# nkb-tech/nkb-classification

Hardware: AMD Instinct MI355X
Metric: images/sec train step (3x224x224) (higher is better)
Workload: dtype bf16; 1 GPU; resnet50 single-task train step, 1000 classes, bs=256/GPU, bf16 compute + fp32 master weights, NAdam, 3x224x224; global_batch=256, parallelism=dp1

## Files before the change

nkb-classification_amd/csrc/elementwise.hip:

```cpp
#include "common.h"
#include <stdlib.h>
#include <atomic>

static inline unsigned grid_for(size_t work_items, int block = 256, unsigned cap = 256 * 16) {
    size_t g = (work_items + block - 1) / block;
    if (g > cap) g = cap;
    if (g < 1) g = 1;
    return (unsigned)g;
}

template <typename T> struct Chunk;
template <> struct Chunk<bf16_t> {
    static constexpr int N = 8;
    typedef u32x4 Raw;
    __device__ static __forceinline__ Raw ldraw(const bf16_t* p) { return *(const u32x4*)p; }
    __device__ static __forceinline__ void unpack(const Raw& r, float* f) { unpack8(r, f); }
    __device__ static __forceinline__ void load(const bf16_t* p, float* f) { unpack8(*(const u32x4*)p, f); }
    __device__ static __forceinline__ void store(bf16_t* p, const float* f) { *(u32x4*)p = pack8(f); }
};
template <> struct Chunk<float> {
    static constexpr int N = 4;
    typedef f32x4 Raw;
    __device__ static __forceinline__ Raw ldraw(const float* p) { return *(const f32x4*)p; }
    __device__ static __forceinline__ void unpack(const Raw& r, float* f) { f[0] = r[0]; f[1] = r[1]; f[2] = r[2]; f[3] = r[3]; }
    __device__ static __forceinline__ void load(const float* p, float* f) {
        const f32x4 v = *(const f32x4*)p;
        f[0] = v[0]; f[1] = v[1]; f[2] = v[2]; f[3] = v[3];
    }
    __device__ static __forceinline__ void store(float* p, const float* f) { *(f32x4*)p = (f32x4){f[0], f[1], f[2], f[3]}; }
};

static inline int env_int(const char* name, int dflt) {
    const char* v = getenv(name);
    return v && *v ? atoi(v) : dflt;
}
#ifndef NKB_BN_FUSED
#define NKB_BN_FUSED 1
#endif
static constexpr int g_bn_fused = NKB_BN_FUSED;

template <int NC>
__device__ __forceinline__ void ldvec(const float* __restrict__ p, float* o) {
#pragma unroll
    for (int i = 0; i < NC / 4; ++i) {
        const f32x4 v = *(const f32x4*)(p + 4 * i);
        o[4 * i] = v[0]; o[4 * i + 1] = v[1]; o[4 * i + 2] = v[2]; o[4 * i + 3] = v[3];
    }
}

static inline int bn_partitions(int C) { return C <= 128 ? 64 : (C <= 256 ? 32 : 16); }
template <bool WT>
__device__ __forceinline__ void bn_partial_reduce_body(const float* __restrict__ partials, int tiles, int C, double* __restrict__ dpart,
                                                       double (&red)[2][16][64]) {
    const int cx = threadIdx.x & 63, py = threadIdx.x >> 6;
    const int c = blockIdx.x * 64 + cx;
    double s = 0.0, ss = 0.0;
    if (c < C) {
        for (int t = blockIdx.y * 16 + py; t < tiles; t += 16 * (int)gridDim.y) {
            s += (double)partials[((size_t)t * 2) * C + c];
            ss += (double)partials[((size_t)t * 2 + 1) * C + c];
        }
    }
    red[0][py][cx] = s;
    red[1][py][cx] = ss;
    __syncthreads();
    if (py != 0 || c >= C) return;
    s = 0.0; ss = 0.0;
    for (int k = 0; k < 16; ++k) { s += red[0][k][cx]; ss += red[1][k][cx]; }
    double* d0 = dpart + ((size_t)blockIdx.y * 2) * C + c;
    double* d1 = dpart + ((size_t)blockIdx.y * 2 + 1) * C + c;
    if constexpr (WT) {
        __hip_atomic_store(d0, s, __ATOMIC_RELAXED, __HIP_MEMORY_SCOPE_AGENT);
        __hip_atomic_store(d1, ss, __ATOMIC_RELAXED, __HIP_MEMORY_SCOPE_AGENT);
    } else {
        *d0 = s; *d1 = ss;
    }
}
__global__ void bn_partial_reduce_kernel(const float* __restrict__ partials, int tiles, int C, double* __restrict__ dpart) {
    __shared__ double red[2][16][64];
    bn_partial_reduce_body<false>(partials, tiles, C, dpart, red);
}

__device__ unsigned g_bn_tickets[128 * 32];
__device__ __forceinline__ bool bn_arrive_last(unsigned* ticket, unsigned parts) {
    __shared__ unsigned last_flag;
    asm volatile("s_waitcnt vmcnt(0)" ::: "memory");
    __syncthreads();
    if (threadIdx.x == 0) {
        const unsigned t = __hip_atomic_fetch_add(ticket, 1u, __ATOMIC_RELAXED, __HIP_MEMORY_SCOPE_AGENT);
        const bool last = t == parts - 1;
        if (last) {
            __hip_atomic_store(ticket, 0u, __ATOMIC_RELAXED, __HIP_MEMORY_SCOPE_AGENT);
            __builtin_amdgcn_fence(__ATOMIC_ACQUIRE, "agent");
            asm volatile("s_waitcnt vmcnt(0)" ::: "memory");
        }
        last_flag = last ? 1u : 0u;
    }
    __syncthreads();
    return last_flag != 0u;
}
static unsigned* bn_ticket_slot(int cols) {
    static std::atomic<unsigned> next{0};
    if (cols > 32) return nullptr;
    unsigned* base = nullptr;
    if (hipGetSymbolAddress((void**)&base, HIP_SYMBOL(g_bn_tickets)) != hipSuccess || !base) return nullptr;
    return base + (next.fetch_add(1u) % 128u) * 32u;
}

template <typename PT>
__device__ __forceinline__ void bn_finalize_body(const PT* __restrict__ partials, int tiles, int C, float count,
                                                 const float* __restrict__ gamma, const float* __restrict__ beta,
                                                 float* __restrict__ running_mean, float* __restrict__ running_var,
                                                 float momentum, float eps, int training, float* __restrict__ scale,
                                                 float* __restrict__ shift, float* __restrict__ save_mean,
                                                 float* __restrict__ save_invstd, double (&red)[2][16][64]) {
    const int cx = threadIdx.x & 63, py = threadIdx.x >> 6;
    const int c = blockIdx.x * 64 + cx;
    double s = 0.0, ss = 0.0;
    if (training && c < C) {
        for (int t = py; t < tiles; t += 16) {
            s += (double)partials[((size_t)t * 2) * C + c];
            ss += (double)partials[((size_t)t * 2 + 1) * C + c];
        }
    }
    red[0][py][cx] = s;
    red[1][py][cx] = ss;
    __syncthreads();
    if (py != 0 || c >= C) return;
    float mean, var;
    if (training) {
        s = 0.0; ss = 0.0;
        for (int k = 0; k < 16; ++k) { s += red[0][k][cx]; ss += red[1][k][cx]; }
        const double m = s / count;
        double v = ss / count - m * m;
        if (v < 0.0) v = 0.0;
        mean = (float)m; var = (float)v;
        const float unbiased = count > 1.f ? (float)(v * count / (count - 1.0)) : var;
        running_mean[c] = (1.f - momentum) * running_mean[c] + momentum * mean;
        running_var[c] = (1.f - momentum) * running_var[c] + momentum * unbiased;
    } else {
        mean = running_mean[c]; var = running_var[c];
    }
    const float invstd = 1.0f / sqrtf(var + eps);
    const float g = gamma ? gamma[c] : 1.f, b = beta ? beta[c] : 0.f;
    scale[c] = g * invstd;
    shift[c] = b - mean * g * invstd;
    if (save_mean) { save_mean[c] = mean; save_invstd[c] = invstd; }
}
template <typename PT>
__global__ void bn_finalize_kernel(const PT* __restrict__ partials, int tiles, int C, float count,
                                   const float* __restrict__ gamma, const float* __restrict__ beta,
                                   float* __restrict__ running_mean, float* __restrict__ running_var,
                                   float momentum, float eps, int training, float* __restrict__ scale,
                                   float* __restrict__ shift, float* __restrict__ save_mean,
                                   float* __restrict__ save_invstd) {
    __shared__ double red[2][16][64];
    bn_finalize_body<PT>(partials, tiles, C, count, gamma, beta, running_mean, running_var, momentum, eps, training, scale, shift,
                         save_mean, save_invstd, red);
}
__global__ __launch_bounds__(1024) void bn_reduce_finalize_kernel(const float* __restrict__ partials, int tiles, int C, double* __restrict__ dpart,
// ... 1276 lines not shown
    const int cx = threadIdx.x & 63, py = threadIdx.x >> 6;
    const int c = blockIdx.x * 64 + cx;
    double a = 0.0, b = 0.0;
    if (c < C) {
        for (int t = py; t < tiles; t += 16) {
            a += (double)partials[((size_t)t * 2) * C + c];
            b += (double)partials[((size_t)t * 2 + 1) * C + c];
        }
    }
    red[0][py][cx] = a;
    red[1][py][cx] = b;
    __syncthreads();
    if (py != 0 || c >= C) return;
    a = 0.0; b = 0.0;
    for (int k = 0; k < 16; ++k) { a += red[0][k][cx]; b += red[1][k][cx]; }
    const float sg = (float)a, sgx = (float)(b * (invstd ? (double)invstd[c] : 1.0));
    sums[c] = sg;
    sums[C + c] = sgx;
    if (dbeta) dbeta[c] += sg;
    if (dgamma) dgamma[c] += sgx;
}
template <typename PT>
__global__ void bn_bwd_finalize_tiles_kernel(const PT* __restrict__ partials, int tiles, int C,
                                             const float* __restrict__ invstd, float* __restrict__ dgamma,
                                             float* __restrict__ dbeta, float* __restrict__ sums) {
    __shared__ double red[2][16][64];
    bn_bwd_finalize_tiles_body<PT>(partials, tiles, C, invstd, dgamma, dbeta, sums, red);
}
__global__ __launch_bounds__(1024) void bn_bwd_reduce_finalize_kernel(const float* __restrict__ stats, int tiles, int C, double* __restrict__ dpart,
                                                                      unsigned* __restrict__ tickets, const float* __restrict__ invstd,
                                                                      float* __restrict__ dgamma, float* __restrict__ dbeta,
                                                                      float* __restrict__ sums) {
    __shared__ double red[2][16][64];
    bn_partial_reduce_body<true>(stats, tiles, C, dpart, red);
    if (!bn_arrive_last(tickets + blockIdx.x, gridDim.y)) return;
    bn_bwd_finalize_tiles_body<double>(dpart, (int)gridDim.y, C, invstd, dgamma, dbeta, sums, red);
}

static void launch_bwd_tile_sums(float* stats, int tiles, int C, const float* invstd, float* dgamma, float* dbeta, float* sums,
                                 hipStream_t stream) {
    double* dpart = (double*)(stats + (((size_t)tiles * 2 * C + 1) & ~(size_t)1));
    const int P = bn_partitions(C);
    unsigned* tickets = g_bn_fused ? bn_ticket_slot((C + 63) / 64) : nullptr;
    if (tickets) {
        hipLaunchKernelGGL(bn_bwd_reduce_finalize_kernel, dim3((C + 63) / 64, P), dim3(1024), 0, stream, stats, tiles, C, dpart, tickets,
                           invstd, dgamma, dbeta, sums);
        return;
    }
    hipLaunchKernelGGL(bn_partial_reduce_kernel, dim3((C + 63) / 64, P), dim3(1024), 0, stream, stats, tiles, C, dpart);
    hipLaunchKernelGGL(bn_bwd_finalize_tiles_kernel<double>, dim3((C + 63) / 64), dim3(1024), 0, stream,
                       (const double*)dpart, P, C, invstd, dgamma, dbeta, sums);
}

int nkb_launch_tile_sums(float* stats, int tiles, int C, float* sums, hipStream_t stream) {
    if (tiles > 128) {
        launch_bwd_tile_sums(stats, tiles, C, nullptr, nullptr, nullptr, sums, stream);
    } else {
        hipLaunchKernelGGL(bn_bwd_finalize_tiles_kernel<float>, dim3((C + 63) / 64), dim3(1024), 0, stream,
                           (const float*)stats, tiles, C, (const float*)nullptr, (float*)nullptr, (float*)nullptr, sums);
    }
    return nkb_check_launch("tile_sums");
}

extern "C" int nkb_bn_backward_from_stats(int dtype, const void* g, const void* x, float* stats, int tiles,
                                          const float* mean, const float* invstd, const float* gamma, long long rows,
                                          int C, float* dgamma, float* dbeta, void* dx, float* sums, hipStream_t stream) {
    const int n = dtype == NKB_DT_BF16 ? 8 : 4;
    if (C % n || rows >= (1ll << 31)) { nkb_set_error("bn_backward_from_stats: unsupported C=%d / rows", C); return 1; }
    {
        NkbProfScope prof(NKB_K_BN_BWD_REDUCE, stream, 0);
        if (tiles > 128) {
            launch_bwd_tile_sums(stats, tiles, C, invstd, dgamma, dbeta, sums, stream);
        } else {
            hipLaunchKernelGGL(bn_bwd_finalize_tiles_kernel<float>, dim3((C + 63) / 64), dim3(1024), 0, stream,
                               (const float*)stats, tiles, C, invstd, dgamma, dbeta, sums);
        }
    }
    if (int rc = nkb_check_launch("bn_bwd_finalize_tiles")) return rc;
    NkbProfScope prof(NKB_K_BN_BWD_APPLY, stream, 0, (double)rows * C * (dtype == NKB_DT_BF16 ? 2 : 4) * 3);
    const unsigned grid = grid_cols((size_t)rows, C / n);
    if (dtype == NKB_DT_BF16)
        hipLaunchKernelGGL(bn_bwd_apply_kernel<bf16_t>, dim3(grid), dim3(256), 0, stream, (const bf16_t*)g, (const bf16_t*)x,
                           (const bf16_t*)nullptr, (const unsigned char*)nullptr, (const float*)nullptr, (const float*)nullptr, mean, invstd, gamma, sums,
                           1.0f / (float)rows, (unsigned)rows, C, (bf16_t*)dx, (bf16_t*)nullptr);
    else
        hipLaunchKernelGGL(bn_bwd_apply_kernel<float>, dim3(grid), dim3(256), 0, stream, (const float*)g, (const float*)x,
                           (const float*)nullptr, (const unsigned char*)nullptr, (const float*)nullptr, (const float*)nullptr, mean, invstd, gamma, sums,
                           1.0f / (float)rows, (unsigned)rows, C, (float*)dx, (float*)nullptr);
    return nkb_check_launch("bn_bwd_apply");
}
```

nkb-classification_amd/csrc/grambn.hip:

```cpp
#include "common.h"
#include "prims.h"
#include <stdlib.h>

template <typename WT> __device__ __forceinline__ float ldw(const WT* p);
template <> __device__ __forceinline__ float ldw<float>(const float* p) { return *p; }
template <> __device__ __forceinline__ float ldw<bf16_t>(const bf16_t* p) { return bf2f(*p); }

int nkb_launch_tile_sums(float* stats, int tiles, int C, float* sums, hipStream_t stream);


template <int C>
__global__ __launch_bounds__(256, 3) void bn_apply_gram_kernel(const bf16_t* __restrict__ c, bf16_t* __restrict__ y,
                                                               const float* __restrict__ scale, const float* __restrict__ shift,
                                                               unsigned rows, float* __restrict__ part) {
    constexpr int CPR = C / 8;
    constexpr int RPS = 256 / CPR;
    constexpr int SR = 8192 / C;
    constexpr int NP = SR / RPS;
    constexpr int NBLK = C / 16, NB = NBLK / 2;
    extern __shared__ __attribute__((aligned(16))) unsigned char smem[];
    const int tid = threadIdx.x, lane = tid & 63, wave = tid >> 6;
    const int wr = wave >> 1, wn = wave & 1;
    const int cc = tid % CPR, srow = tid / CPR;
    float sc[8], sh[8], bsum[8];
    {
        const f32x4 a0 = *(const f32x4*)(scale + cc * 8), a1 = *(const f32x4*)(scale + cc * 8 + 4);
        const f32x4 b0 = *(const f32x4*)(shift + cc * 8), b1 = *(const f32x4*)(shift + cc * 8 + 4);
#pragma unroll
        for (int e = 0; e < 4; ++e) { sc[e] = a0[e]; sc[4 + e] = a1[e]; sh[e] = b0[e]; sh[4 + e] = b1[e]; }
    }
#pragma unroll
    for (int e = 0; e < 8; ++e) bsum[e] = 0.f;
    f32x4 acc[NB][NB];
#pragma unroll
    for (int i = 0; i < NB; ++i)
#pragma unroll
        for (int j = 0; j < NB; ++j) acc[i][j] = (f32x4){0.f, 0.f, 0.f, 0.f};
    const unsigned nstage = (rows + SR - 1) / SR;
    u32x4 ld[NP];
    auto load = [&](unsigned st) {
#pragma unroll
        for (int i = 0; i < NP; ++i) {
            const unsigned r = st * SR + srow + RPS * i;
            ld[i] = (u32x4){0u, 0u, 0u, 0u};
            if (r < rows) ld[i] = *(const u32x4*)(c + (size_t)r * C + cc * 8);
        }
    };
    const int g = lane >> 4, li = lane & 15, q4 = li >> 2, p4 = li & 3;
    unsigned st = blockIdx.x;
    if (st < nstage) load(st);
    for (; st < nstage; st += gridDim.x) {
#pragma unroll
        for (int i = 0; i < NP; ++i) {
            const unsigned r = st * SR + srow + RPS * i;
            float v[8];
            unpack8(ld[i], v);
#pragma unroll
            for (int e = 0; e < 8; ++e) v[e] = fmaxf(v[e] * sc[e] + sh[e], 0.f);
            u32x4 pk = pack8(v);
            if (r < rows) { if (y) *(u32x4*)(y + (size_t)r * C + cc * 8) = pk; }
            else pk = (u32x4){0u, 0u, 0u, 0u};
// ... 183 lines not shown
            }
        }
        __syncthreads();
#pragma unroll
        for (int ii = 0; ii < IC; ++ii) {
            const f32x4 w4 = *(const f32x4*)(wl + (size_t)(i0 + ii < Cin ? i0 + ii : 0) * KR);
            const float w[KR] = {w4[0], w4[1], w4[2], w4[3]};
#pragma unroll
            for (int jj = 0; jj < NJ; ++jj) {
                const int j = tid + 256 * jj;
                const float cv = j < Cin ? cl[(size_t)ii * Cin + j] : 0.f;
#pragma unroll
                for (int k = 0; k < KR; ++k) acc[k][jj] += w[k] * cv;
            }
        }
    }
    float pv[KR], pm[KR];
#pragma unroll
    for (int k = 0; k < KR; ++k) { pv[k] = 0.f; pm[k] = 0.f; }
#pragma unroll
    for (int jj = 0; jj < NJ; ++jj) {
        const int j = tid + 256 * jj;
        if (j < Cin) {
            const float mj = mu[j];
#pragma unroll
            for (int k = 0; k < KR; ++k) {
                if (k0 + k < Cout) T[(size_t)(k0 + k) * Cin + j] = acc[k][jj];
                pv[k] += acc[k][jj] * wl[j * KR + k];
                pm[k] += wl[j * KR + k] * mj;
            }
        }
    }
    float var[KR], mean[KR];
    block_sums<KR>(pv, red, var);
    block_sums<KR>(pm, red, mean);
    if (tid < KR && k0 + tid < Cout) {
        const int c = k0 + tid;
        float v = 0.f, m = 0.f;
#pragma unroll
        for (int k = 0; k < KR; ++k) if (k == tid) { v = var[k]; m = mean[k]; }
        if (v < 0.f) v = 0.f;
        const float unbiased = count > 1.f ? v * (count / (count - 1.f)) : v;
        running_mean[c] = (1.f - momentum) * running_mean[c] + momentum * m;
        running_var[c] = (1.f - momentum) * running_var[c] + momentum * unbiased;
        const float invstd = 1.0f / sqrtf(v + eps);
        const float g = gamma ? gamma[c] : 1.f, b = beta ? beta[c] : 0.f;
        scale[c] = g * invstd;
        shift[c] = b - m * g * invstd;
        save_mean[c] = m;
        save_invstd[c] = invstd;
    }
}

template <typename WT, typename CT, int NJ>
__global__ __launch_bounds__(256) void gram_bwd_coef_kernel(const WT* __restrict__ W, const float* __restrict__ R,
                                                            const float* __restrict__ T, const float* __restrict__ mu,
                                                            const float* __restrict__ gsum, float count, int Cin, int Cout,
                                                            const float* __restrict__ gamma, const float* __restrict__ mean,
                                                            const float* __restrict__ invstd, float* __restrict__ dgamma,
                                                            float* __restrict__ dbeta, float* __restrict__ dW,
                                                            CT* __restrict__ wcat, int ldc, CT* __restrict__ V,
                                                            float* __restrict__ cpart) {
    constexpr int KR = 8;
    __shared__ float red[4 * KR];
    __shared__ float kc[5][KR];
    const int tid = threadIdx.x;
    const int k0 = blockIdx.x * KR;
    float w[KR][NJ], r[KR][NJ], p[KR];
#pragma unroll
    for (int k = 0; k < KR; ++k) {
        p[k] = 0.f;
#pragma unroll
        for (int jj = 0; jj < NJ; ++jj) {
            const int j = tid + 256 * jj;
            const bool ok = j < Cin && k0 + k < Cout;
            w[k][jj] = ok ? ldw<WT>(W + (size_t)(k0 + k) * Cin + j) : 0.f;
            r[k][jj] = ok ? R[(size_t)(k0 + k) * Cin + j] : 0.f;
            p[k] += w[k][jj] * r[k][jj];
        }
    }
    float gc[KR];
    block_sums<KR>(p, red, gc);
    if (tid < KR) {
        const int c = k0 + tid;
        float s = 0.f;
#pragma unroll
        for (int k = 0; k < KR; ++k) if (k == tid) s = gc[k];
        float k1 = 0.f, k2 = 0.f, k3 = 0.f, gb = 0.f;
        if (c < Cout) {
            const float g = gamma ? gamma[c] : 1.f, rs = invstd[c], m = mean[c], db = gsum[c];
            const float dg = rs * (s - m * db);
            k1 = g * rs;
            k2 = -g * rs * rs * dg / count;
            k3 = -g * rs * db / count - k2 * m;
            gb = g * rs * db;
            if (dgamma) dgamma[c] += dg;
            if (dbeta) dbeta[c] += db;
        }
        kc[0][tid] = k1; kc[1][tid] = k2 * count; kc[2][tid] = gb; kc[3][tid] = k2; kc[4][tid] = k3;
    }
    __syncthreads();
#pragma unroll
    for (int jj = 0; jj < NJ; ++jj) {
        const int j = tid + 256 * jj;
        if (j >= Cin) continue;
        const float mj = mu[j];
        float q[KR], cb = 0.f;
#pragma unroll
        for (int k = 0; k < KR; ++k) {
            q[k] = kc[0][k] * w[k][jj];
            cb += kc[4][k] * w[k][jj];
            if (k0 + k < Cout) {
                const size_t o = (size_t)(k0 + k) * Cin + j;
                if (dW) dW[o] += kc[0][k] * r[k][jj] + kc[1][k] * T[o] - kc[2][k] * mj;
                const float v = kc[3][k] * w[k][jj];
                if constexpr (sizeof(CT) == 2) V[o] = f2bf(v); else V[o] = v;
            }
        }
        cpart[(size_t)blockIdx.x * Cin + j] = cb;
        if (wcat == nullptr) continue;
        CT* dst = wcat + (size_t)j * ldc + k0;
        if constexpr (sizeof(CT) == 2) {
            if (k0 + KR <= Cout) *(u32x4*)dst = pack8(q);
            else for (int k = 0; k < KR && k0 + k < Cout; ++k) dst[k] = f2bf(q[k]);
        } else {
            for (int k = 0; k < KR && k0 + k < Cout; ++k) dst[k] = q[k];
        }
    }
}

template <typename WT>
__global__ __launch_bounds__(256) void gram_k1w_kernel(const WT* __restrict__ W, const float* __restrict__ k1, int Cin, int Cout,
                                                       WT* __restrict__ out) {
    __shared__ float tile[64][65];
    const int k0 = blockIdx.x * 64, j0 = blockIdx.y * 64;
    for (int idx = threadIdx.x; idx < 64 * 64; idx += 256) {
        const int k = idx >> 6, j = idx & 63;
        tile[k][j] = (k0 + k < Cout && j0 + j < Cin) ? k1[k0 + k] * ldw<WT>(W + (size_t)(k0 + k) * Cin + j0 + j) : 0.f;
    }
    __syncthreads();
    for (int idx = threadIdx.x; idx < 64 * 64; idx += 256) {
        const int j = idx >> 6, k = idx & 63;
        if (k0 + k < Cout && j0 + j < Cin) {
            WT* d = out + (size_t)(j0 + j) * Cout + k0 + k;
            if constexpr (sizeof(WT) == 2) *d = f2bf(tile[k][j]); else *d = tile[k][j];
        }
    }
}
extern "C" int nkb_gram_k1w(int dtype, const void* w, const float* k1, int Cin, int Cout, void* out, hipStream_t stream) {
    if (dtype != NKB_DT_BF16 && dtype != NKB_DT_F32) { nkb_set_error("gram_k1w: bad dtype %d", dtype); return 1; }
    NkbProfScope prof(NKB_K_WPREP, stream, 0);
    const dim3 grid((Cout + 63) / 64, (Cin + 63) / 64);
    if (dtype == NKB_DT_BF16) hipLaunchKernelGGL(gram_k1w_kernel<bf16_t>, grid, dim3(256), 0, stream, (const bf16_t*)w, k1, Cin, Cout, (bf16_t*)out);
    else hipLaunchKernelGGL(gram_k1w_kernel<float>, grid, dim3(256), 0, stream, (const float*)w, k1, Cin, Cout, (float*)out);
    return nkb_check_launch("gram_k1w");
}

template <typename WT>
__global__ void gram_fold2_kernel(const WT* __restrict__ w1, const float* __restrict__ s1, int K1, const WT* __restrict__ w2,
                                  const float* __restrict__ s2, int K2, int Cout, WT* __restrict__ out, const float* __restrict__ sh1,
                                  const float* __restrict__ sh2, float* __restrict__ shift_out) {
    const int K = K1 + K2;
    const long long n = (long long)Cout * K;
    for (long long i = (long long)blockIdx.x * blockDim.x + threadIdx.x; i < n; i += (long long)gridDim.x * blockDim.x) {
        const int k = (int)(i / K), j = (int)(i - (long long)k * K);
        const float v = j < K1 ? s1[k] * ldw<WT>(w1 + (size_t)k * K1 + j) : s2[k] * ldw<WT>(w2 + (size_t)k * K2 + (j - K1));
        if constexpr (sizeof(WT) == 2) out[i] = f2bf(v); else out[i] = v;
    }
    const int t = blockIdx.x * blockDim.x + threadIdx.x;
    if (t < Cout) shift_out[t] = sh1[t] + sh2[t];
}
extern "C" int nkb_gram_fold2(int dtype, const void* w1, const float* s1, int K1, const void* w2, const float* s2, int K2, int Cout,
                              void* out, const float* shift1, const float* shift2, float* shift_out, hipStream_t stream) {
    if (dtype != NKB_DT_BF16 && dtype != NKB_DT_F32) { nkb_set_error("gram_fold2: bad dtype %d", dtype); return 1; }
    NkbProfScope prof(NKB_K_WPREP, stream, 0);
    const long long n = (long long)Cout * (K1 + K2);
    const unsigned grid = (unsigned)((n + 255) / 256 > 1024 ? 1024 : (n + 255) / 256);
    if (dtype == NKB_DT_BF16)
        hipLaunchKernelGGL(gram_fold2_kernel<bf16_t>, dim3(grid), dim3(256), 0, stream, (const bf16_t*)w1, s1, K1, (const bf16_t*)w2, s2, K2, Cout,
                           (bf16_t*)out, shift1, shift2, shift_out);
    else
        hipLaunchKernelGGL(gram_fold2_kernel<float>, dim3(grid), dim3(256), 0, stream, (const float*)w1, s1, K1, (const float*)w2, s2, K2, Cout,
                           (float*)out, shift1, shift2, shift_out);
    return nkb_check_launch("gram_fold2");
}

__global__ __launch_bounds__(1024) void gram_cbias_kernel(const float* __restrict__ cpart, int nblk, int Cin, float* __restrict__ cbias) {
    __shared__ float red[16][64];
    const int cx = threadIdx.x & 63, py = threadIdx.x >> 6;
    const int j = blockIdx.x * 64 + cx;
    float a = 0.f;
    if (j < Cin)
        for (int b = py; b < nblk; b += 16) a += cpart[(size_t)b * Cin + j];
    red[py][cx] = a;
    __syncthreads();
    if (py == 0 && j < Cin) {
        float t = 0.f;
        for (int k = 0; k < 16; ++k) t += red[k][cx];
        cbias[j] = t;
    }
}

template <typename WT>
static int launch_stats(const void* w, const float* cov, const float* mu, long long count, int Cin, int Cout, const float* gamma,
                        const float* beta, float* rm, float* rv, float momentum, float eps, float* T, float* scale, float* shift,
                        float* mean, float* invstd, hipStream_t stream) {
    const dim3 grid((Cout + 3) / 4), block(256);
    const size_t lds = (size_t)(4 + (Cin <= 256 ? 64 : 32)) * Cin * sizeof(float);
    static bool attr_set = false;
    if (!attr_set) {
        hipFuncSetAttribute((const void*)gram_stats_kernel<WT, 1>, hipFuncAttributeMaxDynamicSharedMemorySize, 80 * 1024);
        hipFuncSetAttribute((const void*)gram_stats_kernel<WT, 2>, hipFuncAttributeMaxDynamicSharedMemorySize, 80 * 1024);
        attr_set = true;
    }
#define NKB_GS(NJ) hipLaunchKernelGGL((gram_stats_kernel<WT, NJ>), grid, block, lds, stream, (const WT*)w, cov, mu, (float)count, Cin, Cout, \
                                      gamma, beta, rm, rv, momentum, eps, T, scale, shift, mean, invstd)
    if (Cin <= 256) NKB_GS(1); else NKB_GS(2);
#undef NKB_GS
    return nkb_check_launch("gram_stats");
}

extern "C" int nkb_gram_bn_stats(int dtype, const void* w, const float* gram, const float* colsum, long long count, int Cin, int Cout,
                                 const float* gamma, const float* beta, float* running_mean, float* running_var, float momentum,
                                 float eps, float* cov, float* mu, float* T, float* scale, float* shift, float* mean, float* invstd,
                                 hipStream_t stream) {
    if ((dtype != NKB_DT_BF16 && dtype != NKB_DT_F32) || Cin < 1 || Cin > 512 || Cin % 4 || Cout < 1 || count < 1) {
        nkb_set_error("gram_bn_stats: unsupported dtype %d / Cin=%d (<= 512, %% 4) / Cout=%d", dtype, Cin, Cout);
        return 1;
    }
    NkbProfScope prof(NKB_K_BN_FINALIZE, stream, 2.0 * Cout * (double)Cin * Cin);
    hipLaunchKernelGGL(gram_cov_kernel, dim3((Cin * Cin + 255) / 256), dim3(256), 0, stream, gram, colsum, 1.0 / (double)count, Cin,
                       cov, mu);
    if (int rc = nkb_check_launch("gram_cov")) return rc;
    if (dtype == NKB_DT_BF16)
        return launch_stats<bf16_t>(w, cov, mu, count, Cin, Cout, gamma, beta, running_mean, running_var, momentum, eps, T, scale, shift,
                                    mean, invstd, stream);
    return launch_stats<float>(w, cov, mu, count, Cin, Cout, gamma, beta, running_mean, running_var, momentum, eps, T, scale, shift, mean,
                               invstd, stream);
}

extern "C" int nkb_gemm_tn_batched(int dtype, const void* a, const void* b, void* out, int M, int Na, int Nb, int lda, int ldb, int ldo,
                                   int outer, int inner, long long sao, long long sai, long long sbo, long long sbi, long long soo,
                                   long long soi, hipStream_t stream);

template <typename WT>
static int launch_bwd(int dtype, const void* w, const float* R, const float* T, const float* mu, const float* gsum, long long count, int Cin,
                      int Cout, const float* gamma, const float* mean, const float* invstd, float* dgamma, float* dbeta, float* dw,
                      void* wcat, void* qsep, float* cbias, float* cpart, void* V, hipStream_t stream) {
    using CT = WT;
    const int ldc = Cout + Cin;
    const int nblk = (Cout + 7) / 8;
    {
        NkbProfScope prof(NKB_K_BN_BWD_REDUCE, stream, 0);
        const dim3 grid(nblk), block(256);
#define NKB_GC(NJ) hipLaunchKernelGGL((gram_bwd_coef_kernel<WT, CT, NJ>), grid, block, 0, stream, (const WT*)w, R, T, mu, gsum, (float)count, \
                                      Cin, Cout, gamma, mean, invstd, dgamma, dbeta, dw, (CT*)wcat, ldc, (CT*)V, cpart)
        if (Cin <= 256) NKB_GC(1); else NKB_GC(2);
#undef NKB_GC
        if (int rc = nkb_check_launch("gram_bwd_coef")) return rc;
        hipLaunchKernelGGL(gram_cbias_kernel, dim3((Cin + 63) / 64), dim3(1024), 0, stream, cpart, nblk, Cin, cbias);
        if (int rc = nkb_check_launch("gram_cbias")) return rc;
    }
    if (qsep) return nkb_gemm_tn_batched(dtype, V, w, qsep, Cout, Cin, Cin, Cin, Cin, Cin, 1, 1, 0, 0, 0, 0, 0, 0, stream);
    return nkb_gemm_tn_batched(dtype, V, w, (CT*)wcat + Cout, Cout, Cin, Cin, Cin, Cin, ldc, 1, 1, 0, 0, 0, 0, 0, 0, stream);
}

extern "C" size_t nkb_gram_bn_backward_workspace_floats(int Cin, int Cout) {
    return (size_t)2 * Cout + (size_t)((Cout + 7) / 8) * Cin + (size_t)Cout * Cin + 64;
}
extern "C" int nkb_gram_bn_backward(int dtype, const void* w, const float* R, const float* T, const float* mu, float* gstats, int tiles,
                                    long long count, int Cin, int Cout, const float* gamma, const float* mean, const float* invstd,
                                    float* dgamma, float* dbeta, float* dw, void* wcat, void* q, float* cbias, float* work,
                                    hipStream_t stream) {
    if ((wcat == nullptr) == (q == nullptr)) { nkb_set_error("gram_bn_backward: exactly one of wcat / q"); return 1; }
    if ((dtype != NKB_DT_BF16 && dtype != NKB_DT_F32) || Cin < 1 || Cin > 512 || Cin % 64 || Cout % 8 || count < 1 || tiles < 1) {
        nkb_set_error("gram_bn_backward: unsupported dtype %d / Cin=%d (<= 512, %% 64) / Cout=%d (%% 8)", dtype, Cin, Cout);
        return 1;
    }
    float* gsum = work;
    float* cpart = work + (((size_t)2 * Cout + 15) & ~(size_t)15);
    void* V = cpart + (((size_t)((Cout + 7) / 8) * Cin + 15) & ~(size_t)15);
    {
        NkbProfScope prof(NKB_K_BN_BWD_REDUCE, stream, 0);
        if (int rc = nkb_launch_tile_sums(gstats, tiles, Cout, gsum, stream)) return rc;
    }
    if (dtype == NKB_DT_BF16)
        return launch_bwd<bf16_t>(dtype, w, R, T, mu, gsum, count, Cin, Cout, gamma, mean, invstd, dgamma, dbeta, dw, wcat, q, cbias, cpart, V, stream);
    return launch_bwd<float>(dtype, w, R, T, mu, gsum, count, Cin, Cout, gamma, mean, invstd, dgamma, dbeta, dw, wcat, q, cbias, cpart, V, stream);
}
```

nkb-classification_amd/csrc/prims.h:

```cpp
#pragma once
#include "common.h"

__device__ __forceinline__ void glds16(const unsigned char* src, unsigned char* dst) {
    __builtin_amdgcn_global_load_lds((const __attribute__((address_space(1))) void*)src,
                                     (__attribute__((address_space(3))) void*)dst, 16, 0, 0);
}

#define NKB_BARRIER()                                \
    do {                                             \
        asm volatile("" ::: "memory");               \
        __builtin_amdgcn_s_barrier();                \
        asm volatile("" ::: "memory");               \
    } while (0)

template <int N> __device__ __forceinline__ void wait_vmcnt() { asm volatile("s_waitcnt vmcnt(%0)" ::"n"(N) : "memory"); }
#define NKB_VMCNT(n) asm volatile("s_waitcnt vmcnt(" #n ")" ::: "memory")
#define NKB_LGKM(n) asm volatile("s_waitcnt lgkmcnt(" #n ")" ::: "memory")

#define LDS_READ_TR16(dst, addr, off) asm volatile("ds_read_b64_tr_b16 %0, %1 offset:%2" : "=v"(dst) : "v"(addr), "n"(off))
#define LDS_READ128(dst, addr, off) asm volatile("ds_read_b128 %0, %1 offset:%2" : "=v"(dst) : "v"(addr), "n"(off))
#define LDS_WAIT_PAIR(n, f) asm volatile("s_waitcnt lgkmcnt(%2)" : "+v"(f[0]), "+v"(f[1]) : "n"(n))
#define LDS_WAIT_QUAD(n, q) asm volatile("s_waitcnt lgkmcnt(" #n ")" : "+v"(q[0][0]), "+v"(q[0][1]), "+v"(q[1][0]), "+v"(q[1][1]))

__device__ __forceinline__ float row16_sum(float v) {
    v += __builtin_bit_cast(float, __builtin_amdgcn_update_dpp(0, __builtin_bit_cast(int, v), 0xB1, 0xf, 0xf, true));
    v += __builtin_bit_cast(float, __builtin_amdgcn_update_dpp(0, __builtin_bit_cast(int, v), 0x4E, 0xf, 0xf, true));
    v += __builtin_bit_cast(float, __builtin_amdgcn_update_dpp(0, __builtin_bit_cast(int, v), 0x141, 0xf, 0xf, true));
    v += __builtin_bit_cast(float, __builtin_amdgcn_update_dpp(0, __builtin_bit_cast(int, v), 0x140, 0xf, 0xf, true));
    return v;
}

__device__ __forceinline__ int swz128(int row, int ch) { return row * 128 + ((ch ^ (row & 7)) << 4); }
__device__ __forceinline__ int swz256(int row, int ch) { return 256 * row + 16 * (ch ^ (((row & 3) << 2) | ((row >> 2) & 3))); }
__device__ __forceinline__ int swz_px8(int px) { return (px & 3) | (((px >> 3) & 1) << 2); }
__device__ __forceinline__ int swz_px4(int px) { return ((px >> 1) & 1) | (((px >> 3) & 1) << 1); }
__device__ __forceinline__ int swz_lin(int byte_off) { return byte_off ^ (((byte_off >> 8) & 7) << 4); }
```

Baseline: 15420 images/sec.

## Fuse gram-BN backward tile sums, coef and cbias into one ticketed kernel; add LDS stats kernel

The gram-BN backward path previously launched a tile-sum reduction, a coefficient kernel and a cbias reduction separately. These are now merged into one 1024-thread kernel that reduces gstats itself. The last-arriving block, chosen by an atomic ticket, does the cross-block cbias sum. The forward stats for Cin 64/128 also get a single LDS-resident kernel that builds the covariance and T and finalizes the BN stats, replacing separate cov and finalize launches. The goal is fewer launches and fewer global round trips, at the cost of added ticket synchronisation, more per-block work and new size and alignment restrictions.

After: 15510 images/sec, median of 6. Within noise of the previous version (+0.6%).

```diff
diff --git a/nkb-classification_amd/csrc/elementwise.hip b/nkb-classification_amd/csrc/elementwise.hip
--- a/nkb-classification_amd/csrc/elementwise.hip
+++ b/nkb-classification_amd/csrc/elementwise.hip
@@ -1,4 +1,5 @@
 #include "common.h"
+#include "prims.h"
 #include <stdlib.h>
 #include <atomic>
 
@@ -82,23 +83,6 @@
 }
 
 __device__ unsigned g_bn_tickets[128 * 32];
-__device__ __forceinline__ bool bn_arrive_last(unsigned* ticket, unsigned parts) {
-    __shared__ unsigned last_flag;
-    asm volatile("s_waitcnt vmcnt(0)" ::: "memory");
-    __syncthreads();
-    if (threadIdx.x == 0) {
-        const unsigned t = __hip_atomic_fetch_add(ticket, 1u, __ATOMIC_RELAXED, __HIP_MEMORY_SCOPE_AGENT);
-        const bool last = t == parts - 1;
-        if (last) {
-            __hip_atomic_store(ticket, 0u, __ATOMIC_RELAXED, __HIP_MEMORY_SCOPE_AGENT);
-            __builtin_amdgcn_fence(__ATOMIC_ACQUIRE, "agent");
-            asm volatile("s_waitcnt vmcnt(0)" ::: "memory");
-        }
-        last_flag = last ? 1u : 0u;
-    }
-    __syncthreads();
-    return last_flag != 0u;
-}
 static unsigned* bn_ticket_slot(int cols) {
     static std::atomic<unsigned> next{0};
     if (cols > 32) return nullptr;
@@ -106,6 +90,7 @@
     if (hipGetSymbolAddress((void**)&base, HIP_SYMBOL(g_bn_tickets)) != hipSuccess || !base) return nullptr;
     return base + (next.fetch_add(1u) % 128u) * 32u;
 }
+unsigned* nkb_bn_ticket_slot(int cols) { return bn_ticket_slot(cols); }
 
 template <typename PT>
 __device__ __forceinline__ void bn_finalize_body(const PT* __restrict__ partials, int tiles, int C, float count,
@@ -1488,16 +1473,6 @@
                        (const double*)dpart, P, C, invstd, dgamma, dbeta, sums);
 }
 
-int nkb_launch_tile_sums(float* stats, int tiles, int C, float* sums, hipStream_t stream) {
-    if (tiles > 128) {
-        launch_bwd_tile_sums(stats, tiles, C, nullptr, nullptr, nullptr, sums, stream);
-    } else {
-        hipLaunchKernelGGL(bn_bwd_finalize_tiles_kernel<float>, dim3((C + 63) / 64), dim3(1024), 0, stream,
-                           (const float*)stats, tiles, C, (const float*)nullptr, (float*)nullptr, (float*)nullptr, sums);
-    }
-    return nkb_check_launch("tile_sums");
-}
-
 extern "C" int nkb_bn_backward_from_stats(int dtype, const void* g, const void* x, float* stats, int tiles,
                                           const float* mean, const float* invstd, const float* gamma, long long rows,
                                           int C, float* dgamma, float* dbeta, void* dx, float* sums, hipStream_t stream) {
diff --git a/nkb-classification_amd/csrc/grambn.hip b/nkb-classification_amd/csrc/grambn.hip
--- a/nkb-classification_amd/csrc/grambn.hip
+++ b/nkb-classification_amd/csrc/grambn.hip
@@ -6,7 +6,7 @@
 template <> __device__ __forceinline__ float ldw<float>(const float* p) { return *p; }
 template <> __device__ __forceinline__ float ldw<bf16_t>(const bf16_t* p) { return bf2f(*p); }
 
-int nkb_launch_tile_sums(float* stats, int tiles, int C, float* sums, hipStream_t stream);
+unsigned* nkb_bn_ticket_slot(int cols);
 
 
 template <int C>
@@ -296,79 +296,258 @@
     }
 }
 
-template <typename WT, typename CT, int NJ>
-__global__ __launch_bounds__(256) void gram_bwd_coef_kernel(const WT* __restrict__ W, const float* __restrict__ R,
-                                                            const float* __restrict__ T, const float* __restrict__ mu,
-                                                            const float* __restrict__ gsum, float count, int Cin, int Cout,
-                                                            const float* __restrict__ gamma, const float* __restrict__ mean,
-                                                            const float* __restrict__ invstd, float* __restrict__ dgamma,
-                                                            float* __restrict__ dbeta, float* __restrict__ dW,
-                                                            CT* __restrict__ wcat, int ldc, CT* __restrict__ V,
-                                                            float* __restrict__ cpart) {
+template <typename WT, int CIN, int KR>
+__global__ __launch_bounds__(256) void gram_stats_lds_kernel(const WT* __restrict__ W, const float* __restrict__ G,
+                                                             const float* __restrict__ s, double inv_count, float count, int Cout,
+                                                             const float* __restrict__ gamma, const float* __restrict__ beta,
+                                                             float* __restrict__ running_mean, float* __restrict__ running_var,
+                                                             float momentum, float eps, float* __restrict__ mu, float* __restrict__ T,
+                                                             float* __restrict__ scale, float* __restrict__ shift,
+                                                             float* __restrict__ save_mean, float* __restrict__ save_invstd) {
+    constexpr int LD = CIN;
+    constexpr int NG = 256 / CIN;
+    constexpr int KPT = (KR + NG - 1) / NG;
+    constexpr int NCH = CIN / 64;
+    constexpr int U = CIN * CIN / 1024;
+    constexpr int WPK = CIN / 64;
+    extern __shared__ __attribute__((aligned(16))) unsigned char smem[];
+    double* md = (double*)smem;
+    float* cl = (float*)(md + CIN);
+    float* wl = cl + CIN * LD;
+    float* redv = wl + KR * CIN;
+    float* redm = redv + KR * WPK;
+    const int tid = threadIdx.x, lane = tid & 63;
+    const int k0 = blockIdx.x * KR;
+    f32x4 v[U];
+#pragma unroll
+    for (int u = 0; u < U; ++u) v[u] = *(const f32x4*)(G + 4 * (size_t)(tid + 256 * ((u + (int)blockIdx.x) & (U - 1))));
+    float rm0 = 0.f, rv0 = 0.f, ga = 1.f, be = 0.f;
+    if (tid < KR && k0 + tid < Cout) {
+        rm0 = running_mean[k0 + tid]; rv0 = running_var[k0 + tid];
+        if (gamma) ga = gamma[k0 + tid];
+        if (beta) be = beta[k0 + tid];
+    }
+    if (tid < CIN) {
+        const double m = (double)s[tid] * inv_count;
+        md[tid] = m;
+        if (blockIdx.x == 0) mu[tid] = (float)m;
+    }
+    for (int idx = tid; idx < KR * CIN; idx += 256) {
+        const int k = idx / CIN, i = idx - k * CIN;
+        wl[i * KR + k] = (k0 + k < Cout) ? ldw<WT>(W + (size_t)(k0 + k) * CIN + i) : 0.f;
+    }
+#pragma unroll
+    for (int u = 0; u < U; ++u) {
+        const int idx = tid + 256 * ((u + (int)blockIdx.x) & (U - 1));
+        *(f32x4*)(cl + 4 * idx) = v[u];
+    }
+    __syncthreads();
+    {
+        constexpr int PB = 8;
+        const int i = tid % CIN;
+        const double mi = md[i];
+        for (int d0 = tid / CIN; d0 <= CIN / 2; d0 += NG * PB) {
+            float a[PB], b[PB];
+            double mj[PB];
+            bool ok[PB];
+#pragma unroll
+            for (int u = 0; u < PB; ++u) {
+                const int d = d0 + NG * u, j = (i + d) % CIN;
+                ok[u] = d < CIN / 2 || (d == CIN / 2 && i < CIN / 2);
+                a[u] = cl[i * LD + j]; b[u] = cl[j * LD + i]; mj[u] = md[j];
+            }
+#pragma unroll
+            for (int u = 0; u < PB; ++u) {
+                const int d = d0 + NG * u, j = (i + d) % CIN;
+                const double g = 0.5 * ((double)a[u] + (double)b[u]);
+                const float c = (float)(g * inv_count - mi * mj[u]);
+                if (ok[u]) { cl[i * LD + j] = c; cl[j * LD + i] = c; }
+            }
+        }
+    }
+    __syncthreads();
+    {
+        const int j = tid % CIN, g = tid / CIN;
+        const int rot = (k0 >> 2) % NCH;
+        float acc[KPT];
+        int kk[KPT];
+#pragma unroll
+        for (int m = 0; m < KPT; ++m) { acc[m] = 0.f; kk[m] = g + NG * m < KR ? g + NG * m : 0; }
+        for (int c = 0; c < NCH; ++c) {
+            const int i0 = ((c + rot) % NCH) * 64;
+            const float* cp = cl + i0 * LD + j;
+            const float* wp = wl + i0 * KR;
+#pragma unroll
+            for (int ii = 0; ii < 64; ++ii) {
+                const float cv = cp[ii * LD];
+#pragma unroll
+                for (int m = 0; m < KPT; ++m) acc[m] += wp[ii * KR + kk[m]] * cv;
+            }
+        }
+#pragma unroll
+        for (int m = 0; m < KPT; ++m) {
+            const int k = g + NG * m;
+            if (k >= KR) break;
+            if (k0 + k < Cout) T[(size_t)(k0 + k) * CIN + j] = acc[m];
+            const float w = wl[j * KR + k];
+            const float pv = wave_sum(acc[m] * w), pm = wave_sum(w * (float)md[j]);
+            if (lane == 0) { redv[k * WPK + (j >> 6)] = pv; redm[k * WPK + (j >> 6)] = pm; }
+        }
+    }
+    __syncthreads();
+    if (tid < KR && k0 + tid < Cout) {
+        const int c = k0 + tid;
+        float var = 0.f, m = 0.f;
+#pragma unroll
+        for (int q = 0; q < WPK; ++q) { var += redv[tid * WPK + q]; m += redm[tid * WPK + q]; }
+        if (var < 0.f) var = 0.f;
+        const float unbiased = count > 1.f ? var * (count / (count - 1.f)) : var;
+        running_mean[c] = (1.f - momentum) * rm0 + momentum * m;
+        running_var[c] = (1.f - momentum) * rv0 + momentum * unbiased;
+        const float invstd = 1.0f / sqrtf(var + eps);
+        scale[c] = ga * invstd;
+        shift[c] = be - m * ga * invstd;
+        save_mean[c] = m;
+        save_invstd[c] = invstd;
+    }
+}
+constexpr size_t gram_stats_lds_bytes(int CIN, int KR) {
+    return (size_t)CIN * 8 + ((size_t)CIN * CIN + (size_t)KR * CIN + 2 * (size_t)KR * (CIN / 64)) * 4;
+}
+
+constexpr int GB_LDS = 2048 + 8 * 16 * 64 * 4;
+template <typename WT>
+__global__ __launch_bounds__(1024) void gram_bwd_kernel(const WT* __restrict__ W, const float* __restrict__ R,
+                                                        const float* __restrict__ T, const float* __restrict__ mu,
+                                                        const float* __restrict__ gstats, int tiles, float count, int Cin, int Cout,
+                                                        const float* __restrict__ gamma, const float* __restrict__ mean,
+                                                        const float* __restrict__ invstd, float* __restrict__ dgamma,
+                                                        float* __restrict__ dbeta, float* __restrict__ dW, WT* __restrict__ wcat,
+                                                        int ldc, WT* __restrict__ V, float* cpart, unsigned* ticket,
+                                                        float* __restrict__ cbias) {
     constexpr int KR = 8;
-    __shared__ float red[4 * KR];
-    __shared__ float kc[5][KR];
-    const int tid = threadIdx.x;
+    extern __shared__ __attribute__((aligned(16))) unsigned char smem[];
+    double* dred = (double*)smem;
+    float* fred = (float*)(smem + 1024);
+    float* kc = (float*)(smem + 1536);
+    unsigned* flag = (unsigned*)(smem + 1792);
+    float* cred = (float*)(smem + 2048);
+    const int tid = threadIdx.x, lane = tid & 63, wave = tid >> 6;
     const int k0 = blockIdx.x * KR;
-    float w[KR][NJ], r[KR][NJ], p[KR];
+    const int j = tid;
+    const bool act = j < Cin;
+    float w[KR], r[KR], tk[KR], dw0[KR];
 #pragma unroll
     for (int k = 0; k < KR; ++k) {
-        p[k] = 0.f;
-#pragma unroll
-        for (int jj = 0; jj < NJ; ++jj) {
-            const int j = tid + 256 * jj;
-            const bool ok = j < Cin && k0 + k < Cout;
-            w[k][jj] = ok ? ldw<WT>(W + (size_t)(k0 + k) * Cin + j) : 0.f;
-            r[k][jj] = ok ? R[(size_t)(k0 + k) * Cin + j] : 0.f;
-            p[k] += w[k][jj] * r[k][jj];
-        }
-    }
-    float gc[KR];
-    block_sums<KR>(p, red, gc);
+        const unsigned o = (unsigned)((k0 + k) * Cin + j);
+        w[k] = act ? ldw<WT>(W + o) : 0.f;
+        r[k] = act ? R[o] : 0.f;
+        tk[k] = (act && dW) ? T[o] : 0.f;
+        dw0[k] = (act && dW) ? dW[o] : 0.f;
+    }
+    const float mj = act ? mu[j] : 0.f;
+    float ga = 1.f, rs = 0.f, mc = 0.f, dg0 = 0.f, db0 = 0.f;
     if (tid < KR) {
         const int c = k0 + tid;
+        if (gamma) ga = gamma[c];
+        rs = invstd[c]; mc = mean[c];
+        if (dgamma) dg0 = dgamma[c];
+        if (dbeta) db0 = dbeta[c];
+    }
+    {
+        double a[4] = {0.0, 0.0, 0.0, 0.0};
+        const float* gp = gstats + k0 + 4 * (tid & 1);
+        constexpr int TB = 8;
+        for (int t0 = tid >> 1; t0 < tiles; t0 += 512 * TB) {
+            f32x4 g4[TB];
+#pragma unroll
+            for (int u = 0; u < TB; ++u) {
+                const int t = t0 + 512 * u;
+                g4[u] = (f32x4){0.f, 0.f, 0.f, 0.f};
+                if (t < tiles) g4[u] = *(const f32x4*)(gp + (unsigned)(t * 2 * Cout));
+            }
+#pragma unroll
+            for (int u = 0; u < TB; ++u)
+#pragma unroll
+                for (int e = 0; e < 4; ++e) a[e] += (double)g4[u][e];
+        }
+#pragma unroll
+        for (int e = 0; e < 4; ++e) {
+#pragma unroll
+            for (int o = 2; o < 64; o <<= 1) a[e] += __shfl_xor(a[e], o, 64);
+        }
+        if (lane < 2) {
+#pragma unroll
+            for (int e = 0; e < 4; ++e) dred[wave * KR + 4 * lane + e] = a[e];
+        }
+    }
+#pragma unroll
+    for (int k = 0; k < KR; ++k) {
+        const float t = wave_sum(w[k] * r[k]);
+        if (lane == 0) fred[wave * KR + k] = t;
+    }
+    __syncthreads();
+    if (tid < KR) {
+        const int c = k0 + tid;
+        double gs = 0.0;
         float s = 0.f;
-#pragma unroll
-        for (int k = 0; k < KR; ++k) if (k == tid) s = gc[k];
-        float k1 = 0.f, k2 = 0.f, k3 = 0.f, gb = 0.f;
-        if (c < Cout) {
-            const float g = gamma ? gamma[c] : 1.f, rs = invstd[c], m = mean[c], db = gsum[c];
-            const float dg = rs * (s - m * db);
-            k1 = g * rs;
-            k2 = -g * rs * rs * dg / count;
-            k3 = -g * rs * db / count - k2 * m;
-            gb = g * rs * db;
-            if (dgamma) dgamma[c] += dg;
-            if (dbeta) dbeta[c] += db;
-        }
-        kc[0][tid] = k1; kc[1][tid] = k2 * count; kc[2][tid] = gb; kc[3][tid] = k2; kc[4][tid] = k3;
-    }
-    __syncthreads();
-#pragma unroll
-    for (int jj = 0; jj < NJ; ++jj) {
-        const int j = tid + 256 * jj;
-        if (j >= Cin) continue;
-        const float mj = mu[j];
+        for (int q = 0; q < 16; ++q) gs += dred[q * KR + tid];
+        s = (fred[0 * KR + tid] + fred[1 * KR + tid]) + (fred[2 * KR + tid] + fred[3 * KR + tid]);
+        for (int q = 4; q < 16; ++q) s += fred[q * KR + tid];
+        const float db = (float)gs;
+        const float dg = rs * (s - mc * db);
+        const float k1 = ga * rs;
+        const float k2 = -ga * rs * rs * dg / count;
+        const float k3 = -ga * rs * db / count - k2 * mc;
+        if (dgamma) dgamma[c] = dg0 + dg;
+        if (dbeta) dbeta[c] = db0 + db;
+        kc[0 * KR + tid] = k1; kc[1 * KR + tid] = k2 * count; kc[2 * KR + tid] = ga * rs * db; kc[3 * KR + tid] = k2; kc[4 * KR + tid] = k3;
+    }
+    __syncthreads();
+    if (act) {
         float q[KR], cb = 0.f;
 #pragma unroll
         for (int k = 0; k < KR; ++k) {
-            q[k] = kc[0][k] * w[k][jj];
-            cb += kc[4][k] * w[k][jj];
-            if (k0 + k < Cout) {
-                const size_t o = (size_t)(k0 + k) * Cin + j;
-                if (dW) dW[o] += kc[0][k] * r[k][jj] + kc[1][k] * T[o] - kc[2][k] * mj;
-                const float v = kc[3][k] * w[k][jj];
-                if constexpr (sizeof(CT) == 2) V[o] = f2bf(v); else V[o] = v;
-            }
-        }
-        cpart[(size_t)blockIdx.x * Cin + j] = cb;
-        if (wcat == nullptr) continue;
-        CT* dst = wcat + (size_t)j * ldc + k0;
-        if constexpr (sizeof(CT) == 2) {
-            if (k0 + KR <= Cout) *(u32x4*)dst = pack8(q);
-            else for (int k = 0; k < KR && k0 + k < Cout; ++k) dst[k] = f2bf(q[k]);
-        } else {
-            for (int k = 0; k < KR && k0 + k < Cout; ++k) dst[k] = q[k];
+            q[k] = kc[0 * KR + k] * w[k];
+            cb += kc[4 * KR + k] * w[k];
+            const unsigned o = (unsigned)((k0 + k) * Cin + j);
+            if (dW) dW[o] = dw0[k] + (kc[0 * KR + k] * r[k] + kc[1 * KR + k] * tk[k] - kc[2 * KR + k] * mj);
+            const float v = kc[3 * KR + k] * w[k];
+            if constexpr (sizeof(WT) == 2) V[o] = f2bf(v); else V[o] = v;
+        }
+        __hip_atomic_store(cpart + (unsigned)(blockIdx.x * Cin + j), cb, __ATOMIC_RELAXED, __HIP_MEMORY_SCOPE_AGENT);
+        if (wcat != nullptr) {
+            WT* dst = wcat + (unsigned)(j * ldc + k0);
+            if constexpr (sizeof(WT) == 2) {
+                *(u32x4*)dst = pack8(q);
+            } else {
+#pragma unroll
+                for (int k = 0; k < KR; ++k) dst[k] = q[k];
+            }
+        }
+    }
+    if (!bn_arrive_last(ticket, gridDim.x, flag)) return;
+
+    {
+        const int nblk = (int)gridDim.x;
+        const int cx = tid & 63, py = tid >> 6;
+        constexpr int NCG = 8;
+        float a[NCG];
+#pragma unroll
+        for (int gi = 0; gi < NCG; ++gi) {
+            a[gi] = 0.f;
+            if (gi * 64 < Cin)
+                for (int b = py; b < nblk; b += 16)
+                    a[gi] += __hip_atomic_load(cpart + (unsigned)(b * Cin + gi * 64 + cx), __ATOMIC_RELAXED, __HIP_MEMORY_SCOPE_AGENT);
+        }
+#pragma unroll
+        for (int gi = 0; gi < NCG; ++gi)
+            if (gi * 64 < Cin) cred[(gi * 16 + py) * 64 + cx] = a[gi];
+        __syncthreads();
+        if (tid < Cin) {
+            float t = 0.f;
+            for (int k = 0; k < 16; ++k) t += cred[((tid >> 6) * 16 + k) * 64 + (tid & 63)];
+            cbias[tid] = t;
         }
     }
 }
@@ -429,22 +608,6 @@
     return nkb_check_launch("gram_fold2");
 }
 
-__global__ __launch_bounds__(1024) void gram_cbias_kernel(const float* __restrict__ cpart, int nblk, int Cin, float* __restrict__ cbias) {
-    __shared__ float red[16][64];
-    const int cx = threadIdx.x & 63, py = threadIdx.x >> 6;
-    const int j = blockIdx.x * 64 + cx;
-    float a = 0.f;
-    if (j < Cin)
-        for (int b = py; b < nblk; b += 16) a += cpart[(size_t)b * Cin + j];
-    red[py][cx] = a;
-    __syncthreads();
-    if (py == 0 && j < Cin) {
-        float t = 0.f;
-        for (int k = 0; k < 16; ++k) t += red[k][cx];
-        cbias[j] = t;
-    }
-}
-
 template <typename WT>
 static int launch_stats(const void* w, const float* cov, const float* mu, long long count, int Cin, int Cout, const float* gamma,
                         const float* beta, float* rm, float* rv, float momentum, float eps, float* T, float* scale, float* shift,
@@ -464,6 +627,27 @@
     return nkb_check_launch("gram_stats");
 }
 
+template <typename WT>
+static int launch_stats_lds(const void* w, const float* gram, const float* colsum, long long count, int Cin, int Cout, const float* gamma,
+                            const float* beta, float* rm, float* rv, float momentum, float eps, float* mu, float* T, float* scale,
+                            float* shift, float* mean, float* invstd, hipStream_t stream) {
+    const int KR = Cout >= 4 * 128 ? 4 : (Cout >= 2 * 128 ? 2 : 1);
+    static bool attr_set = false;
+    if (!attr_set) {
+        hipFuncSetAttribute((const void*)gram_stats_lds_kernel<WT, 128, 1>, hipFuncAttributeMaxDynamicSharedMemorySize, (int)gram_stats_lds_bytes(128, 1));
+        hipFuncSetAttribute((const void*)gram_stats_lds_kernel<WT, 128, 2>, hipFuncAttributeMaxDynamicSharedMemorySize, (int)gram_stats_lds_bytes(128, 2));
+        hipFuncSetAttribute((const void*)gram_stats_lds_kernel<WT, 128, 4>, hipFuncAttributeMaxDynamicSharedMemorySize, (int)gram_stats_lds_bytes(128, 4));
+        attr_set = true;
+    }
+#define NKB_GL(CIN, KR_) hipLaunchKernelGGL((gram_stats_lds_kernel<WT, CIN, KR_>), dim3((Cout + KR_ - 1) / KR_), dim3(256), gram_stats_lds_bytes(CIN, KR_), \
+                                            stream, (const WT*)w, gram, colsum, 1.0 / (double)count, (float)count, Cout, gamma, beta, rm, rv, momentum,      \
+                                            eps, mu, T, scale, shift, mean, invstd)
+    if (Cin == 64) { if (KR == 4) NKB_GL(64, 4); else if (KR == 2) NKB_GL(64, 2); else NKB_GL(64, 1); }
+    else { if (KR == 4) NKB_GL(128, 4); else if (KR == 2) NKB_GL(128, 2); else NKB_GL(128, 1); }
+#undef NKB_GL
+    return nkb_check_launch("gram_stats_lds");
+}
+
 extern "C" int nkb_gram_bn_stats(int dtype, const void* w, const float* gram, const float* colsum, long long count, int Cin, int Cout,
                                  const float* gamma, const float* beta, float* running_mean, float* running_var, float momentum,
                                  float eps, float* cov, float* mu, float* T, float* scale, float* shift, float* mean, float* invstd,
@@ -473,6 +657,13 @@
         return 1;
     }
     NkbProfScope prof(NKB_K_BN_FINALIZE, stream, 2.0 * Cout * (double)Cin * Cin);
+    if ((Cin == 64 || Cin == 128) && ((size_t)gram & 15) == 0) {
+        if (dtype == NKB_DT_BF16)
+            return launch_stats_lds<bf16_t>(w, gram, colsum, count, Cin, Cout, gamma, beta, running_mean, running_var, momentum, eps, mu, T,
+                                            scale, shift, mean, invstd, stream);
+        return launch_stats_lds<float>(w, gram, colsum, count, Cin, Cout, gamma, beta, running_mean, running_var, momentum, eps, mu, T, scale,
+                                       shift, mean, invstd, stream);
+    }
     hipLaunchKernelGGL(gram_cov_kernel, dim3((Cin * Cin + 255) / 256), dim3(256), 0, stream, gram, colsum, 1.0 / (double)count, Cin,
                        cov, mu);
     if (int rc = nkb_check_launch("gram_cov")) return rc;
@@ -488,25 +679,20 @@
                                    long long soi, hipStream_t stream);
 
 template <typename WT>
-static int launch_bwd(int dtype, const void* w, const float* R, const float* T, const float* mu, const float* gsum, long long count, int Cin,
-                      int Cout, const float* gamma, const float* mean, const float* invstd, float* dgamma, float* dbeta, float* dw,
-                      void* wcat, void* qsep, float* cbias, float* cpart, void* V, hipStream_t stream) {
-    using CT = WT;
+static int launch_bwd(int dtype, const void* w, const float* R, const float* T, const float* mu, const float* gstats, int tiles,
+                      long long count, int Cin, int Cout, const float* gamma, const float* mean, const float* invstd, float* dgamma,
+                      float* dbeta, float* dw, void* wcat, void* qsep, float* cbias, float* cpart, void* V, hipStream_t stream) {
     const int ldc = Cout + Cin;
-    const int nblk = (Cout + 7) / 8;
+    unsigned* ticket = nkb_bn_ticket_slot(1);
+    if (!ticket) { nkb_set_error("gram_bn_backward: no ticket slot"); return 1; }
     {
         NkbProfScope prof(NKB_K_BN_BWD_REDUCE, stream, 0);
-        const dim3 grid(nblk), block(256);
-#define NKB_GC(NJ) hipLaunchKernelGGL((gram_bwd_coef_kernel<WT, CT, NJ>), grid, block, 0, stream, (const WT*)w, R, T, mu, gsum, (float)count, \
-                                      Cin, Cout, gamma, mean, invstd, dgamma, dbeta, dw, (CT*)wcat, ldc, (CT*)V, cpart)
-        if (Cin <= 256) NKB_GC(1); else NKB_GC(2);
-#undef NKB_GC
-        if (int rc = nkb_check_launch("gram_bwd_coef")) return rc;
-        hipLaunchKernelGGL(gram_cbias_kernel, dim3((Cin + 63) / 64), dim3(1024), 0, stream, cpart, nblk, Cin, cbias);
-        if (int rc = nkb_check_launch("gram_cbias")) return rc;
+        hipLaunchKernelGGL((gram_bwd_kernel<WT>), dim3(Cout / 8), dim3(1024), GB_LDS, stream, (const WT*)w, R, T, mu, gstats, tiles, (float)count,
+                           Cin, Cout, gamma, mean, invstd, dgamma, dbeta, dw, (WT*)wcat, ldc, (WT*)V, cpart, ticket, cbias);
+        if (int rc = nkb_check_launch("gram_bwd")) return rc;
     }
     if (qsep) return nkb_gemm_tn_batched(dtype, V, w, qsep, Cout, Cin, Cin, Cin, Cin, Cin, 1, 1, 0, 0, 0, 0, 0, 0, stream);
-    return nkb_gemm_tn_batched(dtype, V, w, (CT*)wcat + Cout, Cout, Cin, Cin, Cin, Cin, ldc, 1, 1, 0, 0, 0, 0, 0, 0, stream);
+    return nkb_gemm_tn_batched(dtype, V, w, (WT*)wcat + Cout, Cout, Cin, Cin, Cin, Cin, ldc, 1, 1, 0, 0, 0, 0, 0, 0, stream);
 }
 
 extern "C" size_t nkb_gram_bn_backward_workspace_floats(int Cin, int Cout) {
@@ -517,18 +703,20 @@
                                     float* dgamma, float* dbeta, float* dw, void* wcat, void* q, float* cbias, float* work,
                                     hipStream_t stream) {
     if ((wcat == nullptr) == (q == nullptr)) { nkb_set_error("gram_bn_backward: exactly one of wcat / q"); return 1; }
-    if ((dtype != NKB_DT_BF16 && dtype != NKB_DT_F32) || Cin < 1 || Cin > 512 || Cin % 64 || Cout % 8 || count < 1 || tiles < 1) {
+    if ((dtype != NKB_DT_BF16 && dtype != NKB_DT_F32) || Cin < 1 || Cin > 512 || Cin % 64 || Cout < 8 || Cout % 8 || count < 1 || tiles < 1) {
         nkb_set_error("gram_bn_backward: unsupported dtype %d / Cin=%d (<= 512, %% 64) / Cout=%d (%% 8)", dtype, Cin, Cout);
         return 1;
     }
-    float* gsum = work;
+    if ((size_t)gstats & 15) { nkb_set_error("gram_bn_backward: gstats must be 16-byte aligned"); return 1; }
+    if ((long long)tiles * 2 * Cout >= (1ll << 30) || (long long)Cout * (Cout + Cin) >= (1ll << 30)) {
+        nkb_set_error("gram_bn_backward: tiles=%d x Cout=%d too large", tiles, Cout);
+        return 1;
+    }
     float* cpart = work + (((size_t)2 * Cout + 15) & ~(size_t)15);
     void* V = cpart + (((size_t)((Cout + 7) / 8) * Cin + 15) & ~(size_t)15);
-    {
-        NkbProfScope prof(NKB_K_BN_BWD_REDUCE, stream, 0);
-        if (int rc = nkb_launch_tile_sums(gstats, tiles, Cout, gsum, stream)) return rc;
-    }
     if (dtype == NKB_DT_BF16)
-        return launch_bwd<bf16_t>(dtype, w, R, T, mu, gsum, count, Cin, Cout, gamma, mean, invstd, dgamma, dbeta, dw, wcat, q, cbias, cpart, V, stream);
-    return launch_bwd<float>(dtype, w, R, T, mu, gsum, count, Cin, Cout, gamma, mean, invstd, dgamma, dbeta, dw, wcat, q, cbias, cpart, V, stream);
-}
+        return launch_bwd<bf16_t>(dtype, w, R, T, mu, gstats, tiles, count, Cin, Cout, gamma, mean, invstd, dgamma, dbeta, dw, wcat, q, cbias,
+                                  cpart, V, stream);
+    return launch_bwd<float>(dtype, w, R, T, mu, gstats, tiles, count, Cin, Cout, gamma, mean, invstd, dgamma, dbeta, dw, wcat, q, cbias,
+                             cpart, V, stream);
+}
diff --git a/nkb-classification_amd/csrc/prims.h b/nkb-classification_amd/csrc/prims.h
--- a/nkb-classification_amd/csrc/prims.h
+++ b/nkb-classification_amd/csrc/prims.h
@@ -30,6 +30,27 @@
     return v;
 }
 
+__device__ __forceinline__ bool bn_arrive_last(unsigned* ticket, unsigned parts, unsigned* last_flag) {
+    asm volatile("s_waitcnt vmcnt(0)" ::: "memory");
+    __syncthreads();
+    if (threadIdx.x == 0) {
+        const unsigned t = __hip_atomic_fetch_add(ticket, 1u, __ATOMIC_RELAXED, __HIP_MEMORY_SCOPE_AGENT);
+        const bool last = t == parts - 1;
+        if (last) {
+            __hip_atomic_store(ticket, 0u, __ATOMIC_RELAXED, __HIP_MEMORY_SCOPE_AGENT);
+            __builtin_amdgcn_fence(__ATOMIC_ACQUIRE, "agent");
+            asm volatile("s_waitcnt vmcnt(0)" ::: "memory");
+        }
+        *last_flag = last ? 1u : 0u;
+    }
+    __syncthreads();
+    return *last_flag != 0u;
+}
+__device__ __forceinline__ bool bn_arrive_last(unsigned* ticket, unsigned parts) {
+    __shared__ unsigned last_flag;
+    return bn_arrive_last(ticket, parts, &last_flag);
+}
+
 __device__ __forceinline__ int swz128(int row, int ch) { return row * 128 + ((ch ^ (row & 7)) << 4); }
 __device__ __forceinline__ int swz256(int row, int ch) { return 256 * row + 16 * (ch ^ (((row & 3) << 2) | ((row >> 2) & 3))); }
 __device__ __forceinline__ int swz_px8(int px) { return (px & 3) | (((px >> 3) & 1) << 2); }
```
